# Thealexbarney/VGAudio

Measured on AMD Instinct MI355X. Metric: Msamples/s encoded (GC-ADPCM, 4096 ch) at 1/2/4/8 GPUs; % HBM roofline, higher is better.
Workload: dtype int32; 1 GPU; BASELINE configs[1]: 4096 mono channels x 48 kHz x 60 s GC-ADPCM coefficient search + encode per GPU; parallelism=units sharded x1, channels_per_gpu=4096, samples_per_channel=2880000, bit_exact_channels_checked=0

## Files before the change

include/vgaudio_hip_testing.h:

```cpp
#ifndef VGAUDIO_HIP_TESTING_H
#define VGAUDIO_HIP_TESTING_H

#ifdef __cplusplus
extern "C" {
#endif

int vga_testing_force_open_seams_this_thread(int mode);

int vga_testing_gc_encoder_layout_this_thread(int channels_per_wave);
int vga_testing_gc_coefs_variant_this_thread(int variant);
int vga_testing_gc_encoder_segments_this_thread(int segments);
int vga_testing_gc_encoder_persistent_this_thread(int mode);

int vga_testing_gc_plan_pieces(int cus, int groups, int frames, long long group_frames, int ragged, int *out5);

int vga_testing_gc_encode_stats(unsigned long long *out8, int reset);

void vga_testing_host_pipeline_this_thread(int feeders, int drainers, int chunk_units, int slot_bytes);

void vga_testing_host_pipeline_tail_this_thread(int tail_units);

int vga_testing_plan_buckets(const int *group, const int *length, int n, int max_units, long long max_volume, int longest_first,
                             int *order_out, int *chunk_begin_out, int *chunk_length_out, int *chunk_group_out, int max_chunks);
void vga_testing_buckets_order_this_thread(int order);
void vga_testing_host_transfer_this_thread(int mode);
void vga_testing_host_transfer_piece_bytes_this_thread(int bytes);
void vga_testing_host_compute_lanes_this_thread(int lanes);

enum {
    VGA_TESTING_STEP_CHUNK_COMPUTE = 1,
    VGA_TESTING_STEP_TRANSFER = 2,
    VGA_TESTING_STEP_HCA_STREAM_FRAMES = 3
};
void vga_testing_fail_step_this_thread(int kind, int nth);

int vga_testing_last_pipeline_stats(double *out, int n);

int vga_testing_hca_frames_per_group_this_thread(int frames);

// ... 18 lines not shown
```

vgaudio_amd/_lib.py:

```python
import ctypes as C
import importlib.util
import os

_HERE = os.path.dirname(os.path.abspath(__file__))
SO_PATH = os.environ.get("VGAUDIO_HIP_LIBRARY") or os.path.join(_HERE, "libvgaudio_hip.so")

VGA_OK = 0
VGA_ERR_ARGUMENT = -1
VGA_ERR_OUT_OF_RANGE = -2
VGA_ERR_INVALID_DATA = -3
VGA_ERR_INVALID_OP = -4
VGA_ERR_DEVICE = -5

VGA_TESTING_STEP_CHUNK_COMPUTE = 1
VGA_TESTING_STEP_TRANSFER = 2
VGA_TESTING_STEP_HCA_STREAM_FRAMES = 3


class VgaError(RuntimeError):
    code = None


class ArgumentError(VgaError, ValueError):
    code = VGA_ERR_ARGUMENT
# ... 112 lines not shown
    "vga_wave_write_pcm16": (ci, [i16pp, ci, vp, u8p]),
    "vga_wave_write_pcm16_device": (ci, [vp, i64, ci, vp, vp, vp]),
    "vga_adx_key_from_code": (ci, [C.c_uint64, vp]),
    "vga_adx_key_from_string": (ci, [C.c_char_p, vp]),
    "vga_adx_key_code": (C.c_uint64, [vp]),
    "vga_adx_crypt": (ci, [u8pp, ci, ci, vp, ci, ci]),
    "vga_adx_crypt_device": (ci, [vp, i64, ci, ci, vp, ci, ci, vp]),
    "vga_adx_find_key_device": (ci, [vp, i64, ci, ci, ci, ci, vp, ci, C.POINTER(ci), vp]),
    "vga_hca_key_tables": (ci, [ci, C.c_uint64, u8p, u8p]),
    "vga_hca_crypt": (ci, [u8p, ci, ci, u8p]),
    "vga_hca_find_key": (ci, [vp, u8p, ci, u8p, ci, vp]),
    "vga_hca_find_key_device": (ci, [vp, vp, ci, u8p, ci, vp, vp]),
    "vga_hca_byte_position_counts_device": (ci, [vp, i64, ci, ci, ci, ci, vp, vp]),
    "vga_adx_guess_default_candidates": (ci, [ci, vp, vp, vp, vp]),
    "vga_adx_guess_keys": (ci, [vp, ci, ci, ci, vp, ci, vp, ci, vp, ci, vp]),
    "vga_hca_crypt_device": (ci, [vp, i64, ci, ci, ci, u8p, vp]),
    "vga_release_cached_memory": (None, []),
    "vga_testing_force_open_seams_this_thread": (ci, [ci]),
    "vga_testing_host_pipeline_this_thread": (None, [ci, ci, ci, ci]),
    "vga_testing_gc_encoder_layout_this_thread": (ci, [ci]),
    "vga_testing_gc_coefs_variant_this_thread": (ci, [ci]),
    "vga_testing_gc_encoder_segments_this_thread": (ci, [ci]),
    "vga_testing_gc_encoder_persistent_this_thread": (ci, [ci]),
    "vga_testing_last_pipeline_stats": (ci, [vp, ci]),
    "vga_testing_host_pipeline_tail_this_thread": (None, [ci]),
    "vga_testing_buckets_order_this_thread": (None, [ci]),
    "vga_testing_host_transfer_this_thread": (None, [ci]),
    "vga_testing_host_transfer_piece_bytes_this_thread": (None, [ci]),
    "vga_testing_host_compute_lanes_this_thread": (None, [ci]),
    "vga_testing_fail_step_this_thread": (None, [ci, ci]),
    "vga_testing_poison_allocations": (ci, [ci]),
    "vga_testing_plan_buckets": (ci, [C.POINTER(ci), C.POINTER(ci), ci, ci, C.c_longlong, ci, C.POINTER(ci), C.POINTER(ci), C.POINTER(ci),
                                 C.POINTER(ci), ci]),
    "vga_testing_hca_device_info": (ci, [vp, vp, ci]),
    "vga_testing_hca_decode_classes": (ci, [vp, ci, C.POINTER(ci)]),
    "vga_testing_hca_decode_v_stats": (ci, [C.POINTER(C.c_longlong), ci]),
    "vga_testing_hca_ragged_stats": (ci, [vp, C.POINTER(C.c_longlong), ci]),
    "vga_hca_ragged_layout_for": (ci, [vp, ci, C.POINTER(i64), C.POINTER(i64), vp]),
    "vga_hca_ragged_create": (ci, [vp, ci, C.POINTER(vp)]),
    "vga_hca_ragged_destroy": (None, [vp]),
    "vga_hca_ragged_streams": (ci, [vp]),
    "vga_hca_ragged_totals_of": (ci, [vp, vp]),
    "vga_hca_ragged_offsets": (ci, [vp, C.POINTER(i64), C.POINTER(i64)]),
    "vga_testing_adx_ragged_stats": (ci, [vp, C.POINTER(C.c_longlong), ci]),
    "vga_adx_ragged_layout_for": (ci, [vp, C.POINTER(ci), ci, C.POINTER(i64), C.POINTER(i64), vp]),
    "vga_adx_ragged_create": (ci, [vp, C.POINTER(ci), ci, C.POINTER(vp)]),
# ... 576 lines not shown
```

vgaudio_amd/csrc/common.hpp:

```cpp
#pragma once
#include <hip/hip_runtime.h>
#include <cstdarg>
#include <cstdint>
#include <cstdio>
#include <cstdlib>
#include <cstring>
#include <mutex>
#include <vector>

#include "../../include/vgaudio_hip.h"
#include "poison.hpp"

namespace vga {

void set_error(const char *fmt, ...);
bool take_error_pending();

#define VGA_HIP_TRY(expr)                                                              \
    do {                                                                               \
        hipError_t _e = (expr);                                                        \
        if (_e != hipSuccess) {                                                        \
            vga::set_error("%s failed: %s (%s:%d)", #expr, hipGetErrorString(_e),      \
                           __FILE__, __LINE__);                                        \
            return VGA_ERR_DEVICE;                                                     \
// ... 183 lines not shown
__device__ __forceinline__ void lds_barrier()
{
#if defined(__HIP_DEVICE_COMPILE__)
    asm volatile("s_waitcnt lgkmcnt(0)\n\ts_barrier" ::: "memory");
#endif
}

int require_device();

inline int device_cu_count()
{
    int device = 0, cus = 256;
    if (hipGetDevice(&device) == hipSuccess) (void)hipDeviceGetAttribute(&cus, hipDeviceAttributeMultiprocessorCount, device);
    return cus > 0 ? cus : 256;
}

int force_open_seams();

int encoder_layout();
int coefs_kernel_variant();
int encoder_segments_override();
int encoder_persistent_mode();
int hca_frames_per_group_override();
void note_adx_encode_path(int path);
void note_adx_decode_path(int path);

__host__ __device__ inline bool seam_forced_open(int mode, int channel, int seam)
{
    return mode == 1 || mode == 3 || (mode == 2 && channel % 3 == 0 && seam % 2 == 0);
}

}
```

vgaudio_amd/csrc/gc_encode_kernel.hip:

```cpp
#include "common.hpp"
#include "gc_encode_core.hpp"
#include "gcadpcm_kernels.hpp"
#include "seams.hpp"
#include "gc_plan8.hpp"

#include <cstdio>
#include <cstdlib>

namespace vga {
namespace gc {

constexpr int DPP_QUAD_XOR1 = 0xB1;
constexpr int DPP_QUAD_XOR2 = 0x4E;
constexpr int DPP_ROW_HALF_MIRROR = 0x141;
constexpr int DPP_ROW_MIRROR = 0x140;

template <int CTRL>
__device__ __forceinline__ int dpp(int v)
{
    return __builtin_amdgcn_update_dpp(0, v, CTRL, 0xF, 0xF, true);
}

__device__ __forceinline__ unsigned umin32(unsigned a, unsigned b) { return a < b ? a : b; }

template <class Op>
__device__ __forceinline__ unsigned row16_reduce(unsigned v, Op op)
{
    v = op(v, (unsigned)dpp<DPP_QUAD_XOR1>((int)v));
    v = op(v, (unsigned)dpp<DPP_QUAD_XOR2>((int)v));
    v = op(v, (unsigned)dpp<DPP_ROW_HALF_MIRROR>((int)v));
    v = op(v, (unsigned)dpp<DPP_ROW_MIRROR>((int)v));
    return v;
}


#ifdef VGA_DEBUG_TIMESTAMPS
__device__ unsigned long long g_vga_enc_ts[1 << 16];
extern "C" int vga_debug_encode_timestamps(unsigned long long *out, int n)
{
    return (int)hipMemcpyFromSymbol(out, HIP_SYMBOL(g_vga_enc_ts), (size_t)n * sizeof(unsigned long long));
}
#endif
__device__ unsigned long long g_vga_gc_stats[8];
extern "C" int vga_testing_gc_encode_stats(unsigned long long *out8, int reset)
{
    if (hipDeviceSynchronize() != hipSuccess) return -1;
    if (out8 && hipMemcpyFromSymbol(out8, HIP_SYMBOL(g_vga_gc_stats), 8 * sizeof(unsigned long long)) != hipSuccess) return -1;
#ifdef VGA_GC_STATS
    if (out8) out8[7] = 1;
#else
    if (out8) out8[7] = 0;
#endif
    if (reset) {
        const unsigned long long zero[8] = {0, 0, 0, 0, 0, 0, 0, 0};
        if (hipMemcpyToSymbol(HIP_SYMBOL(g_vga_gc_stats), zero, sizeof zero) != hipSuccess) return -1;
    }
    return 0;
}
constexpr int SW = 2;
constexpr int ENC_THREADS = 64 * (SW + 1);
#ifndef VGA_GC_ENCODER_PRIO
#define VGA_GC_ENCODER_PRIO 3
#endif
#ifndef VGA_GC_HELPER_PRIO
#define VGA_GC_HELPER_PRIO 0
#endif
#ifndef VGA_GC_PERSISTENT_WAVES_PER_EU
#define VGA_GC_PERSISTENT_WAVES_PER_EU 3, 3
#endif
template <int CPW, bool SELF = false>
struct Lay {
    static_assert(!SELF || CPW == 8, "the self-served shape is the (channel, predictor) layout");
    static constexpr int EW = SELF ? 1 : SW;
    static constexpr int CS = CPW * EW;
    static constexpr int TF = 64 / CS;
    static constexpr int THREADS = SELF ? 64 : ENC_THREADS;
    static constexpr int BUFS = SELF ? 1 : 2;
};
template <int CS, int TF>
struct GcTileT {
    struct Slot {
// ... 882 lines not shown
    const bool valid = slot_raw < nch && f0 * 14 < total_samples;
    const int16_t *src = pcm + (rg.order ? rg.pcm_off[ch] : (int64_t)ch * pcm_pitch);
    uint8_t *dst = adpcm + (rg.order ? rg.adpcm_off[ch] : (int64_t)ch * adpcm_pitch);
    const int16_t *cf = coefs + ch * 16;
    const int c0 = cf[2 * pr], c1 = cf[2 * pr + 1];
    const bool coef_ok = (c0 < 0 ? -c0 : c0) + (c1 < 0 ? -c1 : c1) <= 32767;
    int h0 = valid ? seg_state[((int64_t)(k - 1) * nch + ch) * 2] : 0;
    int h1 = valid ? seg_state[((int64_t)(k - 1) * nch + ch) * 2 + 1] : 0;
    const int g2 = valid ? src[f0 * 14 - 2] : 0, g1 = valid ? src[f0 * 14 - 1] : 0;
    bool open = valid;
    int frames_run = 0;
    seam_run<LPC>(src, dst, c0, c1, coef_ok, pr, ch, k, f0, total_samples, seg.frames(k), seg.frames(k), force_open, h0, h1, g2, g1, open, frames_run);
    if (valid && lead) {
        atomicAdd(&g_vga_gc_stats[open ? 1 : 0], 1ull);
        atomicAdd(&g_vga_gc_stats[2], (unsigned long long)frames_run);
        seam_flag[(int64_t)(k - 1) * nch + ch] = open ? 1 : 0;
        if (open) {
            seam_end[(int64_t)(k - 1) * nch + ch] = (int)(((unsigned)h1 << 16) | ((unsigned)h0 & 0xFFFFu));
            atomicMin(&first_open[ch], k);
        }
    }
}

template <int LPC>
__global__ __launch_bounds__(64) void gc_encode_seam_kernel(
    const int16_t *__restrict__ pcm, int64_t pcm_pitch, int nch, int total_samples, const Pieces seg,
    const int16_t *__restrict__ coefs, uint8_t *__restrict__ adpcm, int64_t adpcm_pitch,
    const int16_t *__restrict__ seg_state, int *__restrict__ first_open, int *__restrict__ seam_flag,
    int *__restrict__ seam_end, int force_open, const Ragged rg)
{
    seam_piece<LPC>(blockIdx.x * (64 / LPC) + (threadIdx.x / LPC), blockIdx.y + 1, threadIdx.x, pcm, pcm_pitch, nch, total_samples, seg, coefs, adpcm,
               adpcm_pitch, seg_state, first_open, seam_flag, seam_end, force_open, rg);
}

template <int CPW, bool RAGGED>
__global__ __launch_bounds__(ENC_THREADS) __attribute__((amdgpu_waves_per_eu(VGA_GC_PERSISTENT_WAVES_PER_EU))) void gc_encode_persistent_kernel(
    const int16_t *__restrict__ pcm, int64_t pcm_pitch, int nch, int total_samples, const Pieces seg,
    const int16_t *__restrict__ coefs, const int16_t *__restrict__ hist1,
    const int16_t *__restrict__ hist2, uint8_t *adpcm, int64_t adpcm_pitch, int16_t *seg_state,
    const Ragged rg, int groups, int segments, int *__restrict__ queue, int *__restrict__ seam_count, int *first_open,
    int *seam_flag, int *seam_end, int force_open)
{
    static_assert(CPW == 8, "the seams inside the persistent kernel use the (channel, predictor) layout");
    constexpr int CS = Lay<CPW>::CS;
    __shared__ int s_item;
    __shared__ int s_seam[2];
// ... 32 lines not shown
                if (exists(y + 1) && atomicAdd(&seam_count[(int64_t)y * groups + g], 1) == 1) at_end = y + 1;
            }
            s_seam[0] = at_start;
            s_seam[1] = at_end;
        }
        __syncthreads();
        const int seam_a = s_seam[0], seam_b = s_seam[1];
        if ((seam_a | seam_b) != 0) {
            __threadfence();
            const int wave = threadIdx.x >> 6, lane = threadIdx.x & 63;
            if (wave < SW) {
                const int slot = g * CS + wave * CPW + (lane >> 3);
                if (seam_a)
                    seam_piece<8>(slot, seam_a, lane, pcm, pcm_pitch, nch, total_samples, seg, coefs, adpcm, adpcm_pitch, seg_state,
                               first_open, seam_flag, seam_end, force_open, rg);
                if (seam_b)
                    seam_piece<8>(slot, seam_b, lane, pcm, pcm_pitch, nch, total_samples, seg, coefs, adpcm, adpcm_pitch, seg_state,
                               first_open, seam_flag, seam_end, force_open, rg);
            }
        }
    }
}

template <bool RAGGED>
__global__ __launch_bounds__(64) __attribute__((amdgpu_waves_per_eu(3, 3))) void gc_encode_self_served_kernel(
    const int16_t *__restrict__ pcm, int64_t pcm_pitch, int nch, int total_samples, const Pieces seg,
    const int16_t *__restrict__ coefs, const int16_t *__restrict__ hist1,
    const int16_t *__restrict__ hist2, uint8_t *adpcm, int64_t adpcm_pitch, int16_t *seg_state,
    const Ragged rg, int groups, int items, int segments, int *__restrict__ queue, int *__restrict__ seam_count, int *first_open,
    int *seam_flag, int *seam_end, int force_open)
{
    constexpr int CS = PLAN8_SLOTS;
    static_assert(Lay<8, true>::CS == CS && Lay<8, true>::THREADS == 64, "one wave, eight channel slots");
    const int lane = threadIdx.x;
    const uint32_t *host_items = RAGGED ? rg.items : nullptr;
#ifdef VGA_DEBUG_TIMESTAMPS
    if (lane == 0) g_vga_enc_ts[2 * (blockIdx.x & 32767)] = wall_clock64();
#endif
    for (;;) {
        int item = 0;
        if (lane == 0) item = atomicAdd(queue, 1);
        item = __builtin_amdgcn_readfirstlane(item);
        if (item >= items) {
#ifdef VGA_DEBUG_TIMESTAMPS
            if (lane == 0) g_vga_enc_ts[2 * (blockIdx.x & 32767) + 1] = wall_clock64();
#endif
            return;
        }
        int g, y;
        if (!plan8_item(item, groups, nch, host_items, g, y)) continue;
        gc_encode_piece<false, 8, RAGGED, true>(g, y, pcm, pcm_pitch, nch, total_samples, seg, coefs, hist1, hist2, adpcm, adpcm_pitch,
                                                seg_state, (const int *)nullptr, rg);
        if (segments <= 1) continue;
        __threadfence();
        int at_start = 0, at_end = 0;
        if (lane == 0) {
            const int total_wg = RAGGED ? rg.length[rg.order[g * CS]] : total_samples;
            auto exists = [&](int piece) { return piece < segments && seg.first(piece) * 14 < total_wg; };
            if (exists(y)) {
                if (y >= 1 && atomicAdd(&seam_count[(int64_t)(y - 1) * groups + g], 1) == 1) at_start = y;
                if (exists(y + 1) && atomicAdd(&seam_count[(int64_t)y * groups + g], 1) == 1) at_end = y + 1;
            }
        }
        const int seam_a = __builtin_amdgcn_readfirstlane(at_start), seam_b = __builtin_amdgcn_readfirstlane(at_end);
        if ((seam_a | seam_b) != 0) {
            __threadfence();
            const int slot = g * CS + (lane >> 3);
            if (seam_a)
                seam_piece<8>(slot, seam_a, lane, pcm, pcm_pitch, nch, total_samples, seg, coefs, adpcm, adpcm_pitch, seg_state,
                           first_open, seam_flag, seam_end, force_open, rg);
            if (seam_b)
                seam_piece<8>(slot, seam_b, lane, pcm, pcm_pitch, nch, total_samples, seg, coefs, adpcm, adpcm_pitch, seg_state,
                           first_open, seam_flag, seam_end, force_open, rg);
        }
    }
}

template <int LPC>
__global__ __launch_bounds__(64) void gc_encode_chain_kernel(
    const int16_t *__restrict__ pcm, int64_t pcm_pitch, int nch, int total_samples, const Pieces seg, int segments,
    const int16_t *__restrict__ coefs, uint8_t *__restrict__ adpcm, int64_t adpcm_pitch,
    int16_t *__restrict__ seg_state, int *__restrict__ first_open, const int *__restrict__ seam_flag,
    const int *__restrict__ seam_end, int force_open, const Ragged rg)
{
    const int lane = threadIdx.x;
    const int pr = LPC == 16 ? (lane >> 1) & 7 : lane & 7;
    const bool lead = (lane & (LPC - 1)) == 0;
    const int slot_raw = blockIdx.x * (64 / LPC) + lane / LPC;
    const bool live = slot_raw < nch;
    const int slot = live ? slot_raw : nch - 1;
    const int ch = rg.order ? rg.order[slot] : slot;
    if (rg.order) total_samples = rg.length[ch];
    const int mine = live ? first_open[ch] : SEAM_NONE;
    int kmin = mine;
#pragma unroll
    for (int o = LPC; o < 64; o <<= 1) kmin = imin(kmin, __shfl_xor(kmin, o));
    if (kmin >= segments) return;
    if (live && lead && mine < segments) atomicAdd(&g_vga_gc_stats[5], 1ull);
    int frames_run = 0;
    const int16_t *src = pcm + (rg.order ? rg.pcm_off[ch] : (int64_t)ch * pcm_pitch);
    uint8_t *dst = adpcm + (rg.order ? rg.adpcm_off[ch] : (int64_t)ch * adpcm_pitch);
    const int16_t *cf = coefs + ch * 16;
    const int c0 = cf[2 * pr], c1 = cf[2 * pr + 1];
    const bool coef_ok = (c0 < 0 ? -c0 : c0) + (c1 < 0 ? -c1 : c1) <= 32767;
    bool have = false;
    int v0 = 0, v1 = 0;
    int last_k = 0;
    for (int k = kmin; k < segments; k++) {
        const int64_t f0 = seg.first(k);
        const bool exists = f0 * 14 < total_samples;
        if (!__any(exists)) break;
        last_k = k;
        const bool is_last = seg.first(k + 1) * 14 >= total_samples || k == segments - 1;
        const int64_t idx = (int64_t)(k - 1) * nch + ch;
        const bool flagged = live && exists && seam_flag[idx] != 0;
        const int ended = seam_end[idx];
        const bool ran = live && have && exists;
        bool open = ran;
        int h0 = v0, h1 = v1;
        if (__any(ran)) {
            const int g2 = seg_state[idx * 2], g1 = seg_state[idx * 2 + 1];
            if (ran && lead && is_last) {
                seg_state[idx * 2] = (int16_t)v0;
                seg_state[idx * 2 + 1] = (int16_t)v1;
            }
            seam_run<LPC>(src, dst, c0, c1, coef_ok, pr, ch, k, f0, total_samples, seg.frames(k), seg.frames(k), force_open, h0, h1, g2, g1, open, frames_run);
        }
        if (!exists) {
        } else if (ran && open) {
            v0 = h0;
            v1 = h1;
        } else if (flagged) {
            have = true;
            v0 = (int)(int16_t)(ended & 0xFFFF);
            v1 = ended >> 16;
        } else
            have = false;
    }
    if (__any(live && have && total_samples % 14 != 0))
        encode_tail_frame<LPC>(src, dst, c0, c1, coef_ok, pr, total_samples, v0, v1, live && have && total_samples % 14 != 0);
    (void)last_k;
    if (live && lead && frames_run) atomicAdd(&g_vga_gc_stats[2], (unsigned long long)frames_run);
    if (live && lead) first_open[ch] = SEAM_NONE;
}

constexpr int MIN_PIECE_FRAMES = 3584;

constexpr int RAGGED_OVERSUBSCRIPTION = 4;
constexpr int PERSISTENT_MIN_GROUPS_FACTOR = 32;
constexpr int PERSISTENT_SCHEDULE_GROUPS_FACTOR = 8;
constexpr int PERSISTENT_ITEMS_PER_WORKGROUP = 4;
constexpr int PERSISTENT_BIG_ROUNDS = 3;
constexpr int PERSISTENT_SMALL_ROUNDS = 2;
constexpr int PERSISTENT_SMALL_FRAMES = 4096;
constexpr int SELF_SERVED_BIG_ROUNDS = 4;
constexpr int SELF_SERVED_SMALL_ROUNDS = 1;
constexpr int MAX_PIECES = 1024;

static int persistent_wgs_per_cu()
{
// ... 89 lines not shown
    if (RAGGED) sample_count = rg.max_length;
    if (nch <= 0 || sample_count <= 0) return VGA_OK;
    const int groups = (nch + CS - 1) / CS;
    const int cus = device_cu_count();
    const int frames = (sample_count + 13) / 14;
    bool persistent = false;
    Pieces seg;
    int segments;
    const bool want_self = CPW == 8 && self_served_shape(encoder_layout(), groups, cus, RAGGED);
    if (RAGGED && rg.items) {
        persistent = rg.persistent != 0;
        seg = rg.seg;
        segments = rg.segments;
    } else {
        segments = plan_encode_pieces(groups, frames, RAGGED ? rg.total_frames / CS : (int64_t)groups * frames, RAGGED, &persistent, &seg,
                                      want_self ? 1 : CPW);
    }
    const bool self = want_self && persistent;
    const Plan8 p8 = self ? plan_groups_of_eight(cus, nch, segments, RAGGED && rg.items ? rg.n_items : -1) : Plan8{};
    const int seam_groups = self ? p8.groups : groups;
    AsyncBuf scratch;
    int16_t *seg_state = nullptr;
    int *first_open = nullptr, *seam_flag = nullptr, *seam_end = nullptr, *queue = nullptr, *seam_count = nullptr;
    if (segments > 1 || persistent) {
        const size_t state_bytes = segments > 1 ? (size_t)round_up((int64_t)segments * nch * 2 * (int64_t)sizeof(int16_t), 16) : 0;
        const size_t open_bytes = (size_t)round_up((int64_t)nch * (int64_t)sizeof(int), 16);
        const size_t count_bytes = persistent && segments > 1 ? (size_t)round_up((int64_t)(segments - 1) * seam_groups * (int64_t)sizeof(int), 16) : 0;
        const size_t need = 3 * state_bytes + open_bytes + 16 + count_bytes;
        unsigned char *base = static_cast<unsigned char *>(d_scratch);
        if (!base || scratch_bytes < need) {
            VGA_HIP_TRY(scratch.alloc(need, stream));
            base = scratch.as<unsigned char>();
        }
        seam_flag = reinterpret_cast<int *>(base + state_bytes);
        seam_end = reinterpret_cast<int *>(base + 2 * state_bytes);
        first_open = reinterpret_cast<int *>(base + 3 * state_bytes);
        queue = reinterpret_cast<int *>(base + 3 * state_bytes + open_bytes);
        if (segments > 1) {
            seg_state = reinterpret_cast<int16_t *>(base);
            VGA_HIP_TRY(fill_no_open_seams(first_open, nch, stream));
        } else
            seg_state = nullptr;
        seam_count = queue + 4;
        if (persistent) VGA_HIP_TRY(hipMemsetAsync(queue, 0, 16 + count_bytes, stream));
    }
    if (self) {
        if constexpr (CPW == 8)
            hipLaunchKernelGGL((gc_encode_self_served_kernel<RAGGED>), dim3(p8.wgs), dim3(Lay<8, true>::THREADS), 0, stream, d_pcm, pcm_pitch,
                               nch, sample_count, seg, d_coefs, d_hist1, d_hist2, d_adpcm, adpcm_pitch, seg_state, rg, p8.groups, p8.items,
                               segments, queue, seam_count, first_open, seam_flag, seam_end, force_open_seams());
    } else if (persistent) {
        const int items = RAGGED && rg.items ? rg.n_items : groups * segments;
        const int wgs = imin(items, cus * persistent_wgs_per_cu());
        if constexpr (CPW == 8)
            hipLaunchKernelGGL((gc_encode_persistent_kernel<CPW, RAGGED>), dim3(wgs), dim3(ENC_THREADS), 0, stream, d_pcm, pcm_pitch, nch,
                               sample_count, seg, d_coefs, d_hist1, d_hist2, d_adpcm, adpcm_pitch, seg_state, rg, groups, segments, queue,
                               seam_count, first_open, seam_flag, seam_end, force_open_seams());
    } else
        hipLaunchKernelGGL((gc_encode_kernel<false, CPW, RAGGED>), dim3(groups, segments), dim3(ENC_THREADS), 0, stream, d_pcm, pcm_pitch, nch,
                           sample_count, seg, d_coefs, d_hist1, d_hist2, d_adpcm, adpcm_pitch, seg_state,
                           (const int *)nullptr, rg);
    VGA_HIP_TRY(hipGetLastError());
    if (segments > 1) {
        if (!persistent) {
#ifdef VGA_GC_SEAM16_ALWAYS
            const bool wide = CPW == 4;
#else
            const bool wide = CPW == 4 && nch > 64;
#endif
            if (wide)
                hipLaunchKernelGGL(gc_encode_seam_kernel<16>, dim3((nch + 3) / 4, segments - 1), dim3(64), 0, stream, d_pcm, pcm_pitch, nch,
                                   sample_count, seg, d_coefs, d_adpcm, adpcm_pitch, seg_state, first_open, seam_flag, seam_end,
                                   force_open_seams(), rg);
            else
                hipLaunchKernelGGL(gc_encode_seam_kernel<8>, dim3((nch + 7) / 8, segments - 1), dim3(64), 0, stream, d_pcm, pcm_pitch, nch,
                                   sample_count, seg, d_coefs, d_adpcm, adpcm_pitch, seg_state, first_open, seam_flag, seam_end,
                                   force_open_seams(), rg);
            VGA_HIP_TRY(hipGetLastError());
        }
#ifdef VGA_GC_SEAM16_ALWAYS
        if (CPW == 4)
#else
        if (CPW == 4 && nch > 64)
#endif
            hipLaunchKernelGGL(gc_encode_chain_kernel<16>, dim3((nch + 3) / 4), dim3(64), 0, stream, d_pcm, pcm_pitch, nch, sample_count,
                               seg, segments, d_coefs, d_adpcm, adpcm_pitch, seg_state, first_open, seam_flag, seam_end,
                               force_open_seams(), rg);
        else
            hipLaunchKernelGGL(gc_encode_chain_kernel<8>, dim3((nch + 7) / 8), dim3(64), 0, stream, d_pcm, pcm_pitch, nch, sample_count,
                               seg, segments, d_coefs, d_adpcm, adpcm_pitch, seg_state, first_open, seam_flag, seam_end,
                               force_open_seams(), rg);
        VGA_HIP_TRY(hipGetLastError());
        hipLaunchKernelGGL((gc_encode_kernel<true, CPW, RAGGED>), dim3(groups, 1), dim3(ENC_THREADS), 0, stream, d_pcm, pcm_pitch, nch, sample_count,
                           seg, d_coefs, d_hist1, d_hist2, d_adpcm, adpcm_pitch, seg_state, (const int *)first_open, rg);
        VGA_HIP_TRY(hipGetLastError());
    }
    return VGA_OK;
}

size_t encode_scratch_bytes(int nch) { return (size_t)(nch > 0 ? nch : 0) * (1024 * 12 + 4 + 512) + 8192; }

int launch_encode(const int16_t *d_pcm, int64_t pcm_pitch, int nch, int sample_count, const int16_t *d_coefs,
                  const int16_t *d_hist1, const int16_t *d_hist2, uint8_t *d_adpcm, int64_t adpcm_pitch,
                  hipStream_t stream, void *d_scratch, size_t scratch_bytes, const Ragged *rg)
{
    if (rg)
        return launch_encode_layout<8, true>(d_pcm, 0, nch, 0, d_coefs, d_hist1, d_hist2, d_adpcm, 0, stream, d_scratch,
                                             scratch_bytes, *rg);
    int layout = encoder_layout();
    if (layout == 0)
        layout = encoder_persistent_mode() != 2 && ((nch + 15) / 16) * PERSISTENT_MIN_GROUPS_FACTOR < device_cu_count() * 4 ? 4 : 8;
    if (layout == 4)
        return launch_encode_layout<4, false>(d_pcm, pcm_pitch, nch, sample_count, d_coefs, d_hist1, d_hist2, d_adpcm, adpcm_pitch, stream,
                                              d_scratch, scratch_bytes, Ragged{});
    return launch_encode_layout<8, false>(d_pcm, pcm_pitch, nch, sample_count, d_coefs, d_hist1, d_hist2, d_adpcm, adpcm_pitch, stream,
                                          d_scratch, scratch_bytes, Ragged{});
}

}
}
```

vgaudio_amd/csrc/gc_plan8.hpp:

```cpp
#pragma once
#include <cstdint>

#if defined(__HIPCC__)
#define VGA_PLAN8_HD __host__ __device__
#else
#define VGA_PLAN8_HD
#endif

namespace vga {
namespace gc {

constexpr int PLAN8_SLOTS = 8;
constexpr int PLAN8_WGS_PER_CU = 12;

struct Plan8 {
    int groups = 0;
    int items = 0;
    int wgs = 0;
    int rounds_x16 = 0;
};

inline Plan8 plan_groups_of_eight(int cus, int nch, int segments, int host_items)
{
    Plan8 p;
    if (nch <= 0 || segments <= 0 || cus <= 0) return p;
    p.groups = (nch + PLAN8_SLOTS - 1) / PLAN8_SLOTS;
    p.items = host_items >= 0 ? 2 * host_items : p.groups * segments;
    const int cap = cus * PLAN8_WGS_PER_CU;
    p.wgs = p.items < cap ? p.items : cap;
    p.rounds_x16 = p.wgs > 0 ? (int)(((int64_t)p.items * 16 + p.wgs - 1) / p.wgs) : 0;
    return p;
}

VGA_PLAN8_HD inline bool plan8_item(int item, int groups8, int nch, const uint32_t *host_items, int &g, int &y)
{
    if (host_items) {
        const uint32_t v = host_items[item >> 1];
        g = 2 * (int)(v & 0xFFFFFu) + (item & 1);
        y = (int)(v >> 20);
    } else {
        g = item % groups8;
        y = item / groups8;
    }
    return g * PLAN8_SLOTS < nch;
}

}
}
```

vgaudio_amd/csrc/host_batch.hpp:

```cpp
#pragma once
#include <algorithm>
#include <atomic>
#include <cstdlib>
#include <memory>
#include <mutex>
#include "common.hpp"
#include "host_pipeline.hpp"
#include "../../include/vgaudio_hip_testing.h"

namespace vga {

struct PipeOverride {
    int feeders = 0, drainers = 0, chunk_units = 0, slot_bytes = 0, tail_units = 0;
    int buckets_order = 0;
    int transfer = 0;
    int piece_bytes = 0;
    int compute_lanes = 0;
};
struct FailStep {
    int kind = 0, nth = 0, seen = 0;
};
constexpr const char *kRefusedStep = "step refused by vga_testing_fail_step_this_thread";
int launch_transfer(const pipe::Job::TransferPiece *pieces, int n, hipStream_t stream);
int device_cu_count();

struct ThreadSettings {
    int force_open_seams = 0;
    int encoder_layout = 0;
    int coefs_variant = 0;
    int encoder_segments = 0;
    int encoder_persistent = 0;
    int hca_frames_per_group = 0;
    PipeOverride pipe;
    FailStep fail;
};
ThreadSettings &thread_settings();
inline PipeOverride &pipe_override() { return thread_settings().pipe; }
inline bool refuse_step(int kind)
{
    FailStep &f = thread_settings().fail;
    return f.kind == kind && ++f.seen == f.nth;
}
struct PipeReport { pipe::Stats stats; double t_alloc = 0, t_entry = 0; };
PipeReport &pipe_report();
int hardware_queues_requested();
inline int planned_compute_lanes(int own_choice)
{
    const int hook = pipe_override().compute_lanes;
    return std::max(1, std::min(hook > 0 ? hook : own_choice, pipe::kMaxComputeLanes));
}

std::vector<int> batch_devices();

struct ProgressCallback { void (*fn)(void *user, int64_t done, int64_t total) = nullptr; void *user = nullptr; };
ProgressCallback progress_callback();
// ... 321 lines not shown
```

vgaudio_amd/csrc/runtime.hip:

```cpp
#include "common.hpp"
#include "host_batch.hpp"
#include "../../include/vgaudio_hip_testing.h"

namespace vga {

static thread_local char g_err[512] = "";
static thread_local bool g_err_pending = false;

void set_error(const char *fmt, ...)
{
    va_list ap;
    va_start(ap, fmt);
    vsnprintf(g_err, sizeof g_err, fmt, ap);
    va_end(ap);
    g_err_pending = true;
}

bool take_error_pending()
{
    const bool was = g_err_pending;
    g_err_pending = false;
    return was;
}

int require_device()
{
    g_err_pending = false;
    int n = 0;
    hipError_t e = hipGetDeviceCount(&n);
    if (e != hipSuccess || n <= 0) {
        set_error("no HIP device available (%s); libvgaudio_hip has no CPU fallback",
                  e == hipSuccess ? "device count 0" : hipGetErrorString(e));
        return VGA_ERR_DEVICE;
    }
    return VGA_OK;
}

static thread_local ThreadSettings g_settings;
ThreadSettings &thread_settings() { return g_settings; }
int force_open_seams() { return g_settings.force_open_seams; }
int encoder_layout() { return g_settings.encoder_layout; }
int coefs_kernel_variant() { return g_settings.coefs_variant; }
int encoder_segments_override() { return g_settings.encoder_segments; }
int encoder_persistent_mode() { return g_settings.encoder_persistent; }
int hca_frames_per_group_override() { return g_settings.hca_frames_per_group; }
static thread_local int g_adx_encode_path = 0, g_adx_decode_path = 0;
void note_adx_encode_path(int path) { g_adx_encode_path = path; }
void note_adx_decode_path(int path) { g_adx_decode_path = path; }

static int g_queues_seen_by_runtime = 4;
__attribute__((constructor)) static void read_hardware_queues()
{
    if (const char *host = std::getenv("GPU_MAX_HW_QUEUES"))
        g_queues_seen_by_runtime = std::atoi(host);
}
int hardware_queues_requested() { return g_queues_seen_by_runtime; }

static std::mutex g_devices_mutex;
static std::vector<int> g_devices;
std::vector<int> batch_devices()
{
    std::lock_guard<std::mutex> g(g_devices_mutex);
    return g_devices;
}

static thread_local PipeReport g_pipe_report;
PipeReport &pipe_report() { return g_pipe_report; }
static thread_local ProgressCallback g_progress_callback;
// ... 69 lines not shown
int vga_testing_gc_encoder_layout_this_thread(int channels_per_wave)
{
    const int old = g_settings.encoder_layout;
    if (channels_per_wave == 0 || channels_per_wave == 1 || channels_per_wave == 4 || channels_per_wave == 8)
        g_settings.encoder_layout = channels_per_wave;
    return old;
}
int vga_testing_gc_coefs_variant_this_thread(int variant)
{
    const int old = g_settings.coefs_variant;
    if (variant >= 0 && variant <= 3) g_settings.coefs_variant = variant;
    return old;
}
int vga_testing_gc_encoder_segments_this_thread(int segments)
{
    const int old = g_settings.encoder_segments;
    g_settings.encoder_segments = segments > 0 ? segments : 0;
    return old;
}
int vga_testing_gc_encoder_persistent_this_thread(int mode)
{
    const int old = g_settings.encoder_persistent;
    g_settings.encoder_persistent = mode >= 0 && mode <= 2 ? mode : 0;
    return old;
}
int vga_testing_hca_frames_per_group_this_thread(int frames)
{
    const int old = g_settings.hca_frames_per_group;
    g_settings.hca_frames_per_group = frames > 0 ? frames : 0;
    return old;
}
int vga_testing_adx_last_path_this_thread(int *encode, int *decode)
{
    if (encode) *encode = g_adx_encode_path;
    if (decode) *decode = g_adx_decode_path;
    return 0;
}
void vga_testing_host_pipeline_this_thread(int feeders, int drainers, int chunk_units, int slot_bytes)
{
    PipeOverride &o = g_settings.pipe;
    o.feeders = feeders;
    o.drainers = drainers;
    o.chunk_units = chunk_units;
    o.slot_bytes = slot_bytes;
}
void vga_testing_host_pipeline_tail_this_thread(int tail_units) { g_settings.pipe.tail_units = tail_units > 0 ? tail_units : 0; }
// ... 44 lines not shown
```

vgaudio_amd/signals.py:

```python
import numpy as np

from . import synth

CLASSES = ("sine440", "white_full_scale", "noise_3lsb", "silence", "clipped_square", "slow_channel_93")
SINE_PERIOD = 1200
_M32 = 0xFFFFFFFF


def sine_table():
    i = np.arange(SINE_PERIOD, dtype=np.float64)
    return (32767.0 * np.sin(2.0 * np.pi * 440.0 * i / 48000.0)).astype(np.int16)


def _hash32_np(c, i):
    idx = (i.astype(np.uint64) + c.astype(np.uint64) * np.uint64(0x9E3779B1)) & np.uint64(_M32)
    h = (idx * np.uint64(0x85EBCA77)) & np.uint64(_M32)
    h ^= h >> np.uint64(15)
    h = (h * np.uint64(0xC2B2AE3D)) & np.uint64(_M32)
    h ^= h >> np.uint64(13)
    h = (h * np.uint64(0x27D4EB2F)) & np.uint64(_M32)
    h ^= h >> np.uint64(16)
    return h


def host(cls, nch, n, first_channel=0):
    c = (np.arange(nch, dtype=np.int64) + first_channel)[:, None]
    i = np.arange(n, dtype=np.int64)[None, :]
    if cls == "sine440":
        return sine_table()[(i + 37 * c) % SINE_PERIOD]
    if cls == "white_full_scale":
        return ((_hash32_np(c, i) & np.uint64(0xFFFF)).astype(np.int64) - 32768).astype(np.int16)
    if cls == "noise_3lsb":
        return ((_hash32_np(c, i) % np.uint64(7)).astype(np.int64) - 3).astype(np.int16)
    if cls == "silence":
        return np.zeros((nch, n), dtype=np.int16)
    if cls == "clipped_square":
        p = 32 + c % 97
        return np.where((i % p) < p // 2, 32767, -32768).astype(np.int16)
    if cls == "slow_channel_93":
        return np.repeat(synth.generate(1, n, first_channel=93), nch, axis=0)
    raise ValueError(cls)


def device(cls, nch, n, dev, first_channel=0, out=None, chunk=32):
    import torch

    from . import device as vdev
    if out is None:
        out = vdev.alloc_pcm(nch, n, dev)
    if cls == "silence":
        out.zero_()
        return out
    if cls == "slow_channel_93":
        row = vdev.synth_pcm(1, n, dev, first_channel=93)
        out[:, :row.shape[1]] = row
        return out
    i = torch.arange(n, dtype=torch.int64, device=dev)[None, :]
    table = torch.from_numpy(sine_table()).to(dev) if cls == "sine440" else None
    for c0 in range(0, nch, chunk):
        c1 = min(c0 + chunk, nch)
        c = (torch.arange(c0, c1, dtype=torch.int64, device=dev) + first_channel)[:, None]
        if cls == "sine440":
            v = table[(i + 37 * c) % SINE_PERIOD]
        elif cls == "clipped_square":
            p = 32 + c % 97
            v = torch.where((i % p) < p // 2, 32767, -32768).to(torch.int16)
# ... 12 lines not shown
```

Baseline: 85220 Msamples/s.

## Hand over seam chains between self-served encoder waves and schedule slow groups first

The self-served GC encoder now resolves seam chains inside the kernel. The second wave to reach a seam takes over the predictor history through per-seam atomic handover words, so the chain kernel can skip channels whose seams were already resolved. A small kernel also ranks channel groups whose coefficients predict slow-settling seams and places them first in the work-item order, which is meant to reduce tail imbalance. This adds scratch memory, extra atomics and fences, and more code paths where correctness can break.

```diff
diff --git a/include/vgaudio_hip_testing.h b/include/vgaudio_hip_testing.h
--- a/include/vgaudio_hip_testing.h
+++ b/include/vgaudio_hip_testing.h
@@ -15,6 +15,11 @@
 int vga_testing_gc_plan_pieces(int cus, int groups, int frames, long long group_frames, int ragged, int *out5);
 
 int vga_testing_gc_encode_stats(unsigned long long *out8, int reset);
+int vga_testing_gc_encode_stats_n(unsigned long long *out, int n, int reset);
+
+int vga_testing_gc_seam_handover_this_thread(int on);
+int vga_testing_gc_slow_order_host(const short *coefs, int nch, int *order);
+int vga_testing_gc_slow_order_device(const void *d_coefs, int nch, int *order);
 
 void vga_testing_host_pipeline_this_thread(int feeders, int drainers, int chunk_units, int slot_bytes);
 
diff --git a/vgaudio_amd/_lib.py b/vgaudio_amd/_lib.py
--- a/vgaudio_amd/_lib.py
+++ b/vgaudio_amd/_lib.py
@@ -158,6 +158,10 @@
     "vga_testing_gc_coefs_variant_this_thread": (ci, [ci]),
     "vga_testing_gc_encoder_segments_this_thread": (ci, [ci]),
     "vga_testing_gc_encoder_persistent_this_thread": (ci, [ci]),
+    "vga_testing_gc_seam_handover_this_thread": (ci, [ci]),
+    "vga_testing_gc_slow_order_host": (ci, [vp, ci, vp]),
+    "vga_testing_gc_slow_order_device": (ci, [vp, ci, vp]),
+    "vga_testing_gc_encode_stats_n": (ci, [C.POINTER(C.c_ulonglong), ci, ci]),
     "vga_testing_last_pipeline_stats": (ci, [vp, ci]),
     "vga_testing_host_pipeline_tail_this_thread": (None, [ci]),
     "vga_testing_buckets_order_this_thread": (None, [ci]),
diff --git a/vgaudio_amd/csrc/common.hpp b/vgaudio_amd/csrc/common.hpp
--- a/vgaudio_amd/csrc/common.hpp
+++ b/vgaudio_amd/csrc/common.hpp
@@ -229,6 +229,7 @@
 int encoder_segments_override();
 int encoder_persistent_mode();
 int hca_frames_per_group_override();
+bool gc_seam_handover_off();
 void note_adx_encode_path(int path);
 void note_adx_decode_path(int path);
 
diff --git a/vgaudio_amd/csrc/gc_encode_kernel.hip b/vgaudio_amd/csrc/gc_encode_kernel.hip
--- a/vgaudio_amd/csrc/gc_encode_kernel.hip
+++ b/vgaudio_amd/csrc/gc_encode_kernel.hip
@@ -6,6 +6,7 @@
 
 #include <cstdio>
 #include <cstdlib>
+#include <vector>
 
 namespace vga {
 namespace gc {
@@ -41,22 +42,25 @@
     return (int)hipMemcpyFromSymbol(out, HIP_SYMBOL(g_vga_enc_ts), (size_t)n * sizeof(unsigned long long));
 }
 #endif
-__device__ unsigned long long g_vga_gc_stats[8];
-extern "C" int vga_testing_gc_encode_stats(unsigned long long *out8, int reset)
-{
+constexpr int GC_STATS = 9;
+__device__ unsigned long long g_vga_gc_stats[GC_STATS];
+extern "C" int vga_testing_gc_encode_stats_n(unsigned long long *out, int n, int reset)
+{
+    if (n < 0 || n > GC_STATS) return -1;
     if (hipDeviceSynchronize() != hipSuccess) return -1;
-    if (out8 && hipMemcpyFromSymbol(out8, HIP_SYMBOL(g_vga_gc_stats), 8 * sizeof(unsigned long long)) != hipSuccess) return -1;
+    if (out && n > 0 && hipMemcpyFromSymbol(out, HIP_SYMBOL(g_vga_gc_stats), (size_t)n * sizeof(unsigned long long)) != hipSuccess) return -1;
 #ifdef VGA_GC_STATS
-    if (out8) out8[7] = 1;
+    if (out && n > 7) out[7] = 1;
 #else
-    if (out8) out8[7] = 0;
+    if (out && n > 7) out[7] = 0;
 #endif
     if (reset) {
-        const unsigned long long zero[8] = {0, 0, 0, 0, 0, 0, 0, 0};
+        const unsigned long long zero[GC_STATS] = {};
         if (hipMemcpyToSymbol(HIP_SYMBOL(g_vga_gc_stats), zero, sizeof zero) != hipSuccess) return -1;
     }
     return 0;
 }
+extern "C" int vga_testing_gc_encode_stats(unsigned long long *out8, int reset) { return vga_testing_gc_encode_stats_n(out8, 8, reset); }
 constexpr int SW = 2;
 constexpr int ENC_THREADS = 64 * (SW + 1);
 #ifndef VGA_GC_ENCODER_PRIO
@@ -985,6 +989,112 @@
     }
 }
 
+constexpr int HAND_ARRIVED = 1;
+constexpr int HAND_V = 2;
+constexpr int HAND_EVER = 4;
+struct Handover {
+    int *word = nullptr;
+    int *token = nullptr, *v = nullptr;
+};
+
+__device__ __forceinline__ void self_served_seams(
+    const int g, const int seam_a, const int seam_b, const int lane, const int groups, const int segments,
+    const int16_t *__restrict__ pcm, int64_t pcm_pitch, int nch, int total_samples, const Pieces seg,
+    const int16_t *__restrict__ coefs, uint8_t *adpcm, int64_t adpcm_pitch,
+    const int16_t *seg_state, int *first_open, int *seam_flag, int *seam_end, int force_open, const Handover hand)
+{
+    const int pr = lane & 7;
+    const bool lead = pr == 0;
+    const int slot_raw = g * PLAN8_SLOTS + (lane >> 3);
+    const bool live = slot_raw < nch;
+    const int ch = live ? slot_raw : nch - 1;
+    const int16_t *src = pcm + (int64_t)ch * pcm_pitch;
+    uint8_t *dst = adpcm + (int64_t)ch * adpcm_pitch;
+    const int16_t *cf = coefs + ch * 16;
+    const int c0 = cf[2 * pr], c1 = cf[2 * pr + 1];
+    const bool coef_ok = (c0 < 0 ? -c0 : c0) + (c1 < 0 ? -c1 : c1) <= 32767;
+    auto second_on = [&](int piece) {
+        __threadfence();
+        int old = 0;
+        if (lane == 0) old = atomicAdd(&hand.word[(int64_t)(piece - 1) * groups + g], 1);
+        const bool second = __builtin_amdgcn_readfirstlane(old) == 1;
+        if (second) __threadfence();
+        return second;
+    };
+    int own = 0;
+    int p = 0;
+    int state = 0, v0 = 0, v1 = 0;
+    for (;;) {
+        const bool cont = p != 0;
+        int k;
+        if (cont) k = p;
+        else if (own == 0) { own = 1; k = seam_a; }
+        else if (own == 1) { own = 2; k = seam_b; }
+        else break;
+        p = 0;
+        if (k == 0) continue;
+        const int64_t f0 = seg.first(k);
+        const bool valid = live && f0 * 14 < total_samples;
+        const int64_t idx = (int64_t)(k - 1) * nch + ch;
+        const int t0 = valid ? seg_state[idx * 2] : 0, t1 = valid ? seg_state[idx * 2 + 1] : 0;
+        int h0 = cont ? v0 : t0, h1 = cont ? v1 : t1;
+        const int g2 = cont ? t0 : (valid ? src[f0 * 14 - 2] : 0), g1 = cont ? t1 : (valid ? src[f0 * 14 - 1] : 0);
+        bool open = cont ? valid && (state & HAND_V) != 0 : valid;
+        const bool ran = open;
+        int frames_run = 0;
+        if (__any(open))
+            seam_run<8>(src, dst, c0, c1, coef_ok, pr, ch, k, f0, total_samples, seg.frames(k), seg.frames(k), force_open, h0, h1, g2, g1, open, frames_run);
+        if (!cont) {
+            if (valid && lead) {
+                atomicAdd(&g_vga_gc_stats[open ? 1 : 0], 1ull);
+                atomicAdd(&g_vga_gc_stats[2], (unsigned long long)frames_run);
+                seam_flag[idx] = open ? 1 : 0;
+                if (open) {
+                    seam_end[idx] = (int)(((unsigned)h1 << 16) | ((unsigned)h0 & 0xFFFFu));
+                    atomicMin(&first_open[ch], k);
+                }
+            }
+            if (!hand.word) continue;
+            if (k == 1) {
+                state = HAND_ARRIVED | (open ? HAND_V | HAND_EVER : 0);
+                v0 = h0;
+                v1 = h1;
+            } else {
+                if (second_on(k)) {
+                    state = hand.token[idx];
+                    const int v = hand.v[idx];
+                    v0 = (int)(int16_t)(v & 0xFFFF);
+                    v1 = v >> 16;
+                    p = k;
+                }
+                continue;
+            }
+        } else {
+            if (valid && lead && frames_run) atomicAdd(&g_vga_gc_stats[2], (unsigned long long)frames_run);
+            const bool flagged = valid && seam_flag[idx] != 0;
+            if (ran && open) {
+                v0 = h0;
+                v1 = h1;
+            } else if (flagged) {
+                const int ended = seam_end[idx];
+                state |= HAND_V | HAND_EVER;
+                v0 = (int)(int16_t)(ended & 0xFFFF);
+                v1 = ended >> 16;
+            } else
+                state &= ~HAND_V;
+        }
+        const bool last = k + 1 >= segments || seg.first(k + 1) * 14 >= total_samples;
+        const int64_t nidx = (int64_t)(last ? segments - 1 : k) * nch + ch;
+        if (live && lead) {
+            hand.v[nidx] = (int)(((unsigned)v1 << 16) | ((unsigned)v0 & 0xFFFFu));
+            hand.token[nidx] = state;
+            if (last && (state & HAND_EVER) != 0) atomicAdd(&g_vga_gc_stats[8], 1ull);
+        }
+        if (last) continue;
+        if (second_on(k + 1)) p = k + 1;
+    }
+}
+
 template <int LPC>
 __global__ __launch_bounds__(64) void gc_encode_seam_kernel(
     const int16_t *__restrict__ pcm, int64_t pcm_pitch, int nch, int total_samples, const Pieces seg,
@@ -1063,18 +1173,71 @@
     }
 }
 
+__global__ __launch_bounds__(64) void gc_slow_groups_kernel(const int16_t *__restrict__ coefs, int nch, int groups8, int *__restrict__ order)
+{
+    const int lane = threadIdx.x;
+    auto flagged = [&](int g) {
+        bool slow = false;
+        if (g < groups8)
+            for (int s = 0; s < PLAN8_SLOTS; s++) {
+                const int ch = g * PLAN8_SLOTS + s;
+                if (ch < nch) slow = plan8_slow_channel(coefs + (int64_t)ch * 16) || slow;
+            }
+        return slow;
+    };
+    int total = 0;
+    for (int base = 0; base < groups8; base += 64) total += __popcll(__ballot(flagged(base + lane)));
+    int s = 0, r = total;
+    const unsigned long long lower = (1ull << lane) - 1;
+    for (int base = 0; base < groups8; base += 64) {
+        const int g = base + lane;
+        const bool f = flagged(g);
+        const unsigned long long m = __ballot(f), rest = __ballot(!f && g < groups8);
+        if (g < groups8) order[f ? s + __popcll(m & lower) : r + __popcll(rest & lower)] = g;
+        s += __popcll(m);
+        r += __popcll(rest);
+    }
+    if (lane == 0) order[groups8] = total;
+}
+extern "C" int vga_testing_gc_slow_order_host(const int16_t *coefs, int nch, int *order)
+{
+    if (!coefs || !order || nch <= 0) return -1;
+    const int groups8 = (nch + PLAN8_SLOTS - 1) / PLAN8_SLOTS;
+    std::vector<unsigned char> flagged((size_t)groups8, 0);
+    for (int ch = 0; ch < nch; ch++)
+        if (plan8_slow_channel(coefs + (int64_t)ch * 16)) flagged[(size_t)(ch / PLAN8_SLOTS)] = 1;
+    return plan8_slow_order(flagged.data(), groups8, order);
+}
+extern "C" int vga_testing_gc_slow_order_device(const void *d_coefs, int nch, int *order)
+{
+    if (!d_coefs || !order || nch <= 0) return -1;
+    const int groups8 = (nch + PLAN8_SLOTS - 1) / PLAN8_SLOTS;
+    int *d_order = nullptr;
+    if (hipMalloc(&d_order, (size_t)(groups8 + 1) * sizeof(int)) != hipSuccess) return -1;
+    hipLaunchKernelGGL(gc_slow_groups_kernel, dim3(1), dim3(64), 0, (hipStream_t)0, static_cast<const int16_t *>(d_coefs), nch, groups8, d_order);
+    std::vector<int> host((size_t)groups8 + 1);
+    const bool ok = hipGetLastError() == hipSuccess &&
+                    hipMemcpy(host.data(), d_order, host.size() * sizeof(int), hipMemcpyDeviceToHost) == hipSuccess;
+    (void)hipFree(d_order);
+    if (!ok) return -1;
+    for (int g = 0; g < groups8; g++) order[g] = host[(size_t)g];
+    return host[(size_t)groups8];
+}
+
 template <bool RAGGED>
 __global__ __launch_bounds__(64) __attribute__((amdgpu_waves_per_eu(3, 3))) void gc_encode_self_served_kernel(
     const int16_t *__restrict__ pcm, int64_t pcm_pitch, int nch, int total_samples, const Pieces seg,
     const int16_t *__restrict__ coefs, const int16_t *__restrict__ hist1,
     const int16_t *__restrict__ hist2, uint8_t *adpcm, int64_t adpcm_pitch, int16_t *seg_state,
     const Ragged rg, int groups, int items, int segments, int *__restrict__ queue, int *__restrict__ seam_count, int *first_open,
-    int *seam_flag, int *seam_end, int force_open)
+    int *seam_flag, int *seam_end, int force_open, const Handover hand, const int *__restrict__ slow_order)
 {
     constexpr int CS = PLAN8_SLOTS;
     static_assert(Lay<8, true>::CS == CS && Lay<8, true>::THREADS == 64, "one wave, eight channel slots");
     const int lane = threadIdx.x;
     const uint32_t *host_items = RAGGED ? rg.items : nullptr;
+    const int *order = RAGGED ? nullptr : slow_order;
+    const int slow = order ? order[groups] : 0;
 #ifdef VGA_DEBUG_TIMESTAMPS
     if (lane == 0) g_vga_enc_ts[2 * (blockIdx.x & 32767)] = wall_clock64();
 #endif
@@ -1089,7 +1252,7 @@
             return;
         }
         int g, y;
-        if (!plan8_item(item, groups, nch, host_items, g, y)) continue;
+        if (!plan8_item(item, groups, nch, host_items, order, slow, segments, g, y)) continue;
         gc_encode_piece<false, 8, RAGGED, true>(g, y, pcm, pcm_pitch, nch, total_samples, seg, coefs, hist1, hist2, adpcm, adpcm_pitch,
                                                 seg_state, (const int *)nullptr, rg);
         if (segments <= 1) continue;
@@ -1106,13 +1269,17 @@
         const int seam_a = __builtin_amdgcn_readfirstlane(at_start), seam_b = __builtin_amdgcn_readfirstlane(at_end);
         if ((seam_a | seam_b) != 0) {
             __threadfence();
-            const int slot = g * CS + (lane >> 3);
-            if (seam_a)
-                seam_piece<8>(slot, seam_a, lane, pcm, pcm_pitch, nch, total_samples, seg, coefs, adpcm, adpcm_pitch, seg_state,
-                           first_open, seam_flag, seam_end, force_open, rg);
-            if (seam_b)
-                seam_piece<8>(slot, seam_b, lane, pcm, pcm_pitch, nch, total_samples, seg, coefs, adpcm, adpcm_pitch, seg_state,
-                           first_open, seam_flag, seam_end, force_open, rg);
+            if constexpr (RAGGED) {
+                const int slot = g * CS + (lane >> 3);
+                if (seam_a)
+                    seam_piece<8>(slot, seam_a, lane, pcm, pcm_pitch, nch, total_samples, seg, coefs, adpcm, adpcm_pitch, seg_state,
+                               first_open, seam_flag, seam_end, force_open, rg);
+                if (seam_b)
+                    seam_piece<8>(slot, seam_b, lane, pcm, pcm_pitch, nch, total_samples, seg, coefs, adpcm, adpcm_pitch, seg_state,
+                               first_open, seam_flag, seam_end, force_open, rg);
+            } else
+                self_served_seams(g, seam_a, seam_b, lane, groups, segments, pcm, pcm_pitch, nch, total_samples, seg, coefs, adpcm,
+                                  adpcm_pitch, seg_state, first_open, seam_flag, seam_end, force_open, hand);
         }
     }
 }
@@ -1122,7 +1289,8 @@
     const int16_t *__restrict__ pcm, int64_t pcm_pitch, int nch, int total_samples, const Pieces seg, int segments,
     const int16_t *__restrict__ coefs, uint8_t *__restrict__ adpcm, int64_t adpcm_pitch,
     int16_t *__restrict__ seg_state, int *__restrict__ first_open, const int *__restrict__ seam_flag,
-    const int *__restrict__ seam_end, int force_open, const Ragged rg)
+    const int *__restrict__ seam_end, int force_open, const Ragged rg, const int *__restrict__ hand_token,
+    const int *__restrict__ hand_v)
 {
     const int lane = threadIdx.x;
     const int pr = LPC == 16 ? (lane >> 1) & 7 : lane & 7;
@@ -1132,12 +1300,20 @@
     const int slot = live ? slot_raw : nch - 1;
     const int ch = rg.order ? rg.order[slot] : slot;
     if (rg.order) total_samples = rg.length[ch];
-    const int mine = live ? first_open[ch] : SEAM_NONE;
-    int kmin = mine;
-#pragma unroll
-    for (int o = LPC; o < 64; o <<= 1) kmin = imin(kmin, __shfl_xor(kmin, o));
-    if (kmin >= segments) return;
-    if (live && lead && mine < segments) atomicAdd(&g_vga_gc_stats[5], 1ull);
+    const int64_t rec_idx = (int64_t)(segments - 1) * nch + ch;
+    const int record = hand_token && live ? hand_token[rec_idx] : 0;
+    const bool resolved = record != 0;
+    const int mine_raw = live ? first_open[ch] : SEAM_NONE;
+    const int mine = resolved ? SEAM_NONE : mine_raw;
+    int kmin = mine, kmin_raw = mine_raw;
+#pragma unroll
+    for (int o = LPC; o < 64; o <<= 1) {
+        kmin = imin(kmin, __shfl_xor(kmin, o));
+        kmin_raw = imin(kmin_raw, __shfl_xor(kmin_raw, o));
+    }
+    if (kmin_raw >= segments) return;
+    const bool tail_left = resolved && (record & HAND_V) != 0 && total_samples % 14 != 0;
+    if (live && lead && (mine < segments || tail_left)) atomicAdd(&g_vga_gc_stats[5], 1ull);
     int frames_run = 0;
     const int16_t *src = pcm + (rg.order ? rg.pcm_off[ch] : (int64_t)ch * pcm_pitch);
     uint8_t *dst = adpcm + (rg.order ? rg.adpcm_off[ch] : (int64_t)ch * adpcm_pitch);
@@ -1154,7 +1330,7 @@
         last_k = k;
         const bool is_last = seg.first(k + 1) * 14 >= total_samples || k == segments - 1;
         const int64_t idx = (int64_t)(k - 1) * nch + ch;
-        const bool flagged = live && exists && seam_flag[idx] != 0;
+        const bool flagged = live && !resolved && exists && seam_flag[idx] != 0;
         const int ended = seam_end[idx];
         const bool ran = live && have && exists;
         bool open = ran;
@@ -1177,6 +1353,12 @@
             v1 = ended >> 16;
         } else
             have = false;
+    }
+    if (tail_left) {
+        const int v = hand_v[rec_idx];
+        have = true;
+        v0 = (int)(int16_t)(v & 0xFFFF);
+        v1 = v >> 16;
     }
     if (__any(live && have && total_samples % 14 != 0))
         encode_tail_frame<LPC>(src, dst, c0, c1, coef_ok, pr, total_samples, v0, v1, live && have && total_samples % 14 != 0);
@@ -1312,11 +1494,15 @@
     AsyncBuf scratch;
     int16_t *seg_state = nullptr;
     int *first_open = nullptr, *seam_flag = nullptr, *seam_end = nullptr, *queue = nullptr, *seam_count = nullptr;
+    const bool handover = self && !RAGGED && segments > 1 && !gc_seam_handover_off();
+    Handover hand;
+    int *slow_order = nullptr;
     if (segments > 1 || persistent) {
         const size_t state_bytes = segments > 1 ? (size_t)round_up((int64_t)segments * nch * 2 * (int64_t)sizeof(int16_t), 16) : 0;
         const size_t open_bytes = (size_t)round_up((int64_t)nch * (int64_t)sizeof(int), 16);
         const size_t count_bytes = persistent && segments > 1 ? (size_t)round_up((int64_t)(segments - 1) * seam_groups * (int64_t)sizeof(int), 16) : 0;
-        const size_t need = 3 * state_bytes + open_bytes + 16 + count_bytes;
+        const size_t order_bytes = handover ? (size_t)round_up((int64_t)(seam_groups + 1) * (int64_t)sizeof(int), 16) : 0;
+        const size_t need = 3 * state_bytes + open_bytes + 16 + count_bytes + (handover ? count_bytes + 2 * state_bytes + order_bytes : 0);
         unsigned char *base = static_cast<unsigned char *>(d_scratch);
         if (!base || scratch_bytes < need) {
             VGA_HIP_TRY(scratch.alloc(need, stream));
@@ -1332,13 +1518,23 @@
         } else
             seg_state = nullptr;
         seam_count = queue + 4;
-        if (persistent) VGA_HIP_TRY(hipMemsetAsync(queue, 0, 16 + count_bytes, stream));
+        if (persistent) VGA_HIP_TRY(hipMemsetAsync(queue, 0, 16 + count_bytes * (handover ? 2 : 1), stream));
+        if (handover) {
+            unsigned char *words = base + 3 * state_bytes + open_bytes + 16 + count_bytes;
+            hand.word = reinterpret_cast<int *>(words);
+            hand.token = reinterpret_cast<int *>(words + count_bytes);
+            hand.v = reinterpret_cast<int *>(words + count_bytes + state_bytes);
+            slow_order = reinterpret_cast<int *>(words + count_bytes + 2 * state_bytes);
+            VGA_HIP_TRY(hipMemsetAsync(hand.token + (size_t)(segments - 1) * nch, 0, (size_t)nch * sizeof(int), stream));
+        }
     }
     if (self) {
-        if constexpr (CPW == 8)
+        if constexpr (CPW == 8) {
+            if (slow_order) hipLaunchKernelGGL(gc_slow_groups_kernel, dim3(1), dim3(64), 0, stream, d_coefs, nch, p8.groups, slow_order);
             hipLaunchKernelGGL((gc_encode_self_served_kernel<RAGGED>), dim3(p8.wgs), dim3(Lay<8, true>::THREADS), 0, stream, d_pcm, pcm_pitch,
                                nch, sample_count, seg, d_coefs, d_hist1, d_hist2, d_adpcm, adpcm_pitch, seg_state, rg, p8.groups, p8.items,
-                               segments, queue, seam_count, first_open, seam_flag, seam_end, force_open_seams());
+                               segments, queue, seam_count, first_open, seam_flag, seam_end, force_open_seams(), hand, (const int *)slow_order);
+        }
     } else if (persistent) {
         const int items = RAGGED && rg.items ? rg.n_items : groups * segments;
         const int wgs = imin(items, cus * persistent_wgs_per_cu());
@@ -1375,11 +1571,11 @@
 #endif
             hipLaunchKernelGGL(gc_encode_chain_kernel<16>, dim3((nch + 3) / 4), dim3(64), 0, stream, d_pcm, pcm_pitch, nch, sample_count,
                                seg, segments, d_coefs, d_adpcm, adpcm_pitch, seg_state, first_open, seam_flag, seam_end,
-                               force_open_seams(), rg);
+                               force_open_seams(), rg, (const int *)hand.token, (const int *)hand.v);
         else
             hipLaunchKernelGGL(gc_encode_chain_kernel<8>, dim3((nch + 7) / 8), dim3(64), 0, stream, d_pcm, pcm_pitch, nch, sample_count,
                                seg, segments, d_coefs, d_adpcm, adpcm_pitch, seg_state, first_open, seam_flag, seam_end,
-                               force_open_seams(), rg);
+                               force_open_seams(), rg, (const int *)hand.token, (const int *)hand.v);
         VGA_HIP_TRY(hipGetLastError());
         hipLaunchKernelGGL((gc_encode_kernel<true, CPW, RAGGED>), dim3(groups, 1), dim3(ENC_THREADS), 0, stream, d_pcm, pcm_pitch, nch, sample_count,
                            seg, d_coefs, d_hist1, d_hist2, d_adpcm, adpcm_pitch, seg_state, (const int *)first_open, rg);
@@ -1388,7 +1584,7 @@
     return VGA_OK;
 }
 
-size_t encode_scratch_bytes(int nch) { return (size_t)(nch > 0 ? nch : 0) * (1024 * 12 + 4 + 512) + 8192; }
+size_t encode_scratch_bytes(int nch) { return (size_t)(nch > 0 ? nch : 0) * (1024 * 20 + 4 + 1024 + 1) + 8192 + 32; }
 
 int launch_encode(const int16_t *d_pcm, int64_t pcm_pitch, int nch, int sample_count, const int16_t *d_coefs,
                   const int16_t *d_hist1, const int16_t *d_hist2, uint8_t *d_adpcm, int64_t adpcm_pitch,
diff --git a/vgaudio_amd/csrc/gc_plan8.hpp b/vgaudio_amd/csrc/gc_plan8.hpp
--- a/vgaudio_amd/csrc/gc_plan8.hpp
+++ b/vgaudio_amd/csrc/gc_plan8.hpp
@@ -32,18 +32,58 @@
     return p;
 }
 
-VGA_PLAN8_HD inline bool plan8_item(int item, int groups8, int nch, const uint32_t *host_items, int &g, int &y)
+#ifndef VGA_PLAN8_SLOW_C1
+#define VGA_PLAN8_SLOW_C1 2040
+#endif
+constexpr int PLAN8_SLOW_C1 = VGA_PLAN8_SLOW_C1;
+VGA_PLAN8_HD inline bool plan8_slow_predictor(int c0, int c1)
+{
+    return -c1 >= PLAN8_SLOW_C1 && (int64_t)c0 * c0 < (int64_t)-8192 * c1;
+}
+VGA_PLAN8_HD inline bool plan8_slow_channel(const int16_t *coefs16)
+{
+    bool slow = false;
+    for (int p = 0; p < 8; p++) slow = slow || plan8_slow_predictor(coefs16[2 * p], coefs16[2 * p + 1]);
+    return slow;
+}
+inline int plan8_slow_order(const unsigned char *flagged, int groups8, int *order)
+{
+    int s = 0;
+    for (int g = 0; g < groups8; g++)
+        if (flagged[g]) order[s++] = g;
+    int r = s;
+    for (int g = 0; g < groups8; g++)
+        if (!flagged[g]) order[r++] = g;
+    return s;
+}
+
+VGA_PLAN8_HD inline bool plan8_item(int item, int groups8, int nch, const uint32_t *host_items, const int *order, int slow, int segments,
+                                    int &g, int &y)
 {
     if (host_items) {
         const uint32_t v = host_items[item >> 1];
         g = 2 * (int)(v & 0xFFFFFu) + (item & 1);
         y = (int)(v >> 20);
+    } else if (order && slow > 0 && slow < groups8) {
+        const int front = slow * segments;
+        if (item < front) {
+            g = order[item % slow];
+            y = item / slow;
+        } else {
+            const int rest = groups8 - slow;
+            g = order[slow + (item - front) % rest];
+            y = (item - front) / rest;
+        }
     } else {
         g = item % groups8;
         y = item / groups8;
     }
     return g * PLAN8_SLOTS < nch;
 }
+VGA_PLAN8_HD inline bool plan8_item(int item, int groups8, int nch, const uint32_t *host_items, int &g, int &y)
+{
+    return plan8_item(item, groups8, nch, host_items, nullptr, 0, 0, g, y);
+}
 
 }
 }
diff --git a/vgaudio_amd/csrc/host_batch.hpp b/vgaudio_amd/csrc/host_batch.hpp
--- a/vgaudio_amd/csrc/host_batch.hpp
+++ b/vgaudio_amd/csrc/host_batch.hpp
@@ -31,6 +31,7 @@
     int encoder_segments = 0;
     int encoder_persistent = 0;
     int hca_frames_per_group = 0;
+    int gc_seam_handover_off = 0;
     PipeOverride pipe;
     FailStep fail;
 };
diff --git a/vgaudio_amd/csrc/runtime.hip b/vgaudio_amd/csrc/runtime.hip
--- a/vgaudio_amd/csrc/runtime.hip
+++ b/vgaudio_amd/csrc/runtime.hip
@@ -44,6 +44,7 @@
 int encoder_segments_override() { return g_settings.encoder_segments; }
 int encoder_persistent_mode() { return g_settings.encoder_persistent; }
 int hca_frames_per_group_override() { return g_settings.hca_frames_per_group; }
+bool gc_seam_handover_off() { return g_settings.gc_seam_handover_off != 0; }
 static thread_local int g_adx_encode_path = 0, g_adx_decode_path = 0;
 void note_adx_encode_path(int path) { g_adx_encode_path = path; }
 void note_adx_decode_path(int path) { g_adx_decode_path = path; }
@@ -159,6 +160,12 @@
 {
     const int old = g_settings.encoder_persistent;
     g_settings.encoder_persistent = mode >= 0 && mode <= 2 ? mode : 0;
+    return old;
+}
+int vga_testing_gc_seam_handover_this_thread(int on)
+{
+    const int old = g_settings.gc_seam_handover_off ? 0 : 1;
+    g_settings.gc_seam_handover_off = on ? 0 : 1;
     return old;
 }
 int vga_testing_hca_frames_per_group_this_thread(int frames)
diff --git a/vgaudio_amd/signals.py b/vgaudio_amd/signals.py
--- a/vgaudio_amd/signals.py
+++ b/vgaudio_amd/signals.py
@@ -42,6 +42,25 @@
     raise ValueError(cls)
 
 
+def tones_in_noise(nch, n, first_channel=0):
+    i = np.arange(n, dtype=np.int64)[None, :]
+    rows = []
+    for c in range(first_channel, first_channel + nch):
+        noise = host("white_full_scale", 1, n, first_channel=c)[0].astype(np.int64)
+        kind = c % 4
+        if kind == 0:
+            amp = 12000 + 100 * (c % 50)
+            row = np.where(((i[0] + c) % 14) < 7, amp, -amp) + noise // 64
+        elif kind == 1:
+            row = (20000.0 * np.sin(2.0 * np.pi * (i[0] + c) / 14.0)).astype(np.int64) + noise // 64
+        elif kind == 2:
+            row = host("sine440", 1, n, first_channel=c)[0].astype(np.int64) // 2 + noise // 256
+        else:
+            row = noise // 8
+        rows.append(row.astype(np.int16))
+    return np.stack(rows)
+
+
 def device(cls, nch, n, dev, first_channel=0, out=None, chunk=32):
     import torch
 
```

Result: faster. 89790 Msamples/s (median of 6 runs) (+5.4%).
